# agussomacal/ROMHighContrast

Measured on AMD Instinct MI355X. Metric: snapshot_solves_per_sec, higher is better.
Workload: dtype f64

## Files before the change

### romhighcontrast_amd/csrc/rom_fem_dev.h

```cpp
#pragma once
#include "rom_fem_plan.h"
#include "rom_mma.h"

struct FemDev {
  int nrb, ncb, N, n1, n1p, nr, nc, nGp, nGa, T, nslots, kblk, npre, nrhs, nexp, ncross, xb0;
  long long dim;
  const double* pool;
  const int* alist;
  const int* aoff;
  int tile_stream;
  const int* pairs;
  int npairs;
  const double* pool_acc;
  const int* wmeta;
  int wp0[5];
  int s1_t0, s1_nterm, s1_ndr;
  const int* s1_items;
  const int* s1_citems;
  const GenTerm* terms;
  const double* Bt;
  const double* P;
  const double* vec;
  const RhsTerm* rhs;
  const PreEdge* pre;
// ... 45 lines not shown
};


FemDev make_dev(const rom_fem* f);

constexpr int S1_COEF_BYTES = 4 * COEF_MAX * 8, S1_WAVE_BYTES = (40 * 64 + 64 * 4 + 64 + 64 + 3 * 64 * 4) * 8;
constexpr int S1_ITEM_PASSES = 4;
constexpr int S1_DENSE_BYTES = 64 * 64 * 8;
constexpr int S1_LDS_BYTES = S1_COEF_BYTES + 4 * S1_WAVE_BYTES + S1_DENSE_BYTES;

__global__ void k_repack_table(const double* __restrict__ G, int ld, int nseg, int n1, int orient, double* __restrict__ Gs);
struct ExtThresholds { unsigned short thr[8]; };
__global__ void k_mask_table(double* __restrict__ G, int ld, int n1, ExtThresholds th);
__global__ void k_build_A0(double* A0, const double* Qp, const double* rho, int n1, int n1p, int N);
__global__ void k_rhs(FemDev f, const double* __restrict__ a);
__global__ void k_coef(FemDev f, const double* __restrict__ a);
__global__ void k_expand(FemDev f, const double* __restrict__ a, int Mc, double* __restrict__ U, long long row0);
__global__ void k_back_pre(FemDev f, const double* __restrict__ a, int Mc);
template <int NS>
__global__ void k_diag_update(FemDev f, const double* __restrict__ a, int slot, int Mc);
__global__ void k_diag_factor(FemDev f, int slot, int j);
__global__ void k_solve1(FemDev f, const double* __restrict__ a, int Mc);
template <int NS>
__global__ void k_factor_panel(FemDev f, const double* __restrict__ a, int j, int Mc);
__global__ void k_backsolve(FemDev f);
__global__ void k_edge_transform(FemDev f, int Mc);
__global__ void k_extend(FemDev f, const double* __restrict__ a, int Mc, double* __restrict__ U, long long row0, const int* __restrict__ blocks, int pw_log2);
struct X128Args {
  int blocks[X128_BLOCKS];
  BlockSide sides[X128_BLOCKS];
};

template <bool FLAT>
__global__ void k_extend128(FemDev f, X128Args xa, const double* __restrict__ a, int Mc, double* __restrict__ U, long long row0, int with_expand, int sys_fast);
__device__ inline void load4_any(const double* __restrict__ p, double v[4]) {
  if (p) {
    v[0] = p[0]; v[1] = p[1]; v[2] = p[2]; v[3] = p[3];
  } else {
    v[0] = v[1] = v[2] = v[3] = 0.0;
  }
}

__device__ inline void expand_tile(const FemDev& f, int Mc, double* __restrict__ U, long long row0, double* lds,
                                   int bx, int by, int bz) {
  if (bz == f.nexp) {
    if (bx != 0) return;
    for (int idx = threadIdx.x; idx < 64 * f.nscat; idx += 256) {
      const int m = by * 64 + idx / f.nscat, v = f.scat[idx % f.nscat];
      if (m < Mc) U[(row0 + m) * f.dim + f.vmap[v]] = f.y[size_t(m) * f.nGp + v];
    }
    return;
  }
  const WavePos wp;
  const ExpEdge ee = f.exp[bz];
  const int srow = stage_row(), sseg = stage_seg();
  const int mA = by * 64 + srow;
  const double* pA = mA < Mc ? f.y + size_t(mA) * f.nGp + ee.zpos + sseg : nullptr;
  const double* pB = f.P + (size_t(ee.ptab) * f.n1p + bx * 64 + srow) * f.n1p + sseg;
  const int kover = ee.zpos < f.nGa ? max(ee.zpos + ee.nch * BK - f.nGa, 0) : 0;
  Acc acc;
  acc_zero(acc);
  gemm_loop(
      ee.nch,
      [&](int ch, double* v) {
        load4_any(pA ? pA + ch * BK : nullptr, v);
        if (kover > 0 && ch == ee.nch - 1) {
#pragma unroll
// ... 33 lines not shown
```

### romhighcontrast_amd/csrc/rom_fem_kernels.hip

```cpp
#include "rom_fem_dev.h"

__global__ void k_build_A0(double* A0, const double* Qp, const double* rho, int n1, int n1p, int N) {
  size_t idx = blockIdx.x * size_t(blockDim.x) + threadIdx.x;
  size_t total = size_t(n1) * n1 * n1p;
  if (idx >= total) return;
  int m = int(idx % n1p);
  size_t ij = idx / n1p;
  int j = int(ij % n1) + 1, i = int(ij / n1) + 1;
  A0[idx] = (m < n1) ? Qp[size_t(j - 1) * n1p + m] * rho[size_t(m) * (N + 1) + i] : 0.0;
}

__global__ void k_repack_table(const double* __restrict__ G, int ld, int nseg, int n1, int orient, double* __restrict__ Gs) {
  const long long idx = blockIdx.x * (long long)blockDim.x + threadIdx.x;
  const long long hrows = (long long)n1 * n1;
  if (idx >= (long long)nseg * hrows * 8) return;
  const int kk = int(idx & 7);
  const long long rp = (idx >> 3) % hrows, seg = (idx >> 3) / hrows;
  const long long row = orient ? (rp % n1) * n1 + rp / n1 : rp;
  const int k = int(seg) * 8 + kk;
  Gs[idx] = k < ld ? G[row * ld + k] : 0.0;
}

__global__ void k_mask_table(double* __restrict__ G, int ld, int n1, ExtThresholds th) {
  const long long idx = blockIdx.x * (long long)blockDim.x + threadIdx.x;
// ... 1436 lines not shown
  const bool odd = wp.lane & 1;
  const int cfirst = acc_col(wp, odd ? 1 : 0) - (odd ? 1 : 0);
  const int ii = i0 + (cfirst >> pw_log2) - 1, jj = j0 + (cfirst & (pw - 1)) - 1;
  const bool v0 = ii < n1 && jj < n1, v1 = ii < n1 && jj + 1 < n1;
  const long long gidx = (long long)(p * N + ii) * f.nc + (q * N + jj);
  double w_own[2];
#pragma unroll
  for (int jb = 0; jb < 2; ++jb) {
    const int cidx = acc_col(wp, jb);
    const int wi = i0 + (cidx >> pw_log2) - 1, wj = j0 + (cidx & (pw - 1)) - 1;
    w_own[jb] = (wi < n1 && wj < n1) ? f.W[wi * n1 + wj] : 0.0;
  }
#pragma unroll
  for (int i = 0; i < 2; ++i)
#pragma unroll
    for (int g = 0; g < 4; ++g) {
      const int m = blockIdx.y * 64 + acc_row(wp, i, g);
      const double sc = scs[acc_row(wp, i, g)];
      const double x0 = acc.c[i][0][g] + sc * w_own[0], x1 = acc.c[i][1][g] + sc * w_own[1];
      const double got = lane_swap1(odd ? x0 : x1);
      if (m >= Mc) continue;
      double* dst = U + (row0 + m) * f.dim + gidx;
      const double lo = odd ? got : x0, hi = odd ? x1 : got;
      if (v1) *reinterpret_cast<double2_u*>(dst) = double2_u{lo, hi};
      else if (v0) dst[0] = lo;
    }
}



constexpr int X128_SLOT = 4 * 128 * 64;
static_assert(sizeof(FemDev) + sizeof(X128Args) + 64 <= 4096, "k_extend128's arguments must fit the kernel argument segment");

__device__ inline int x128_skip(const ExtSide& s, int d) {
  int n = 0;
#pragma unroll
  for (int j = 0; j < EXT_THRESHOLDS; ++j) n += d >= int(s.thr[j]) ? 1 : 0;
  return n;
}

template <bool FLAT>
__global__ __launch_bounds__(512, 2) void k_extend128(FemDev f, X128Args xa, const double* __restrict__ a, int Mc,
                                                      double* __restrict__ U, long long row0, int with_expand,
                                                      int sys_fast) {
  __shared__ __align__(16) char lds_bytes[2 * X128_SLOT];
  __shared__ double scs[128];
  double* const lds = reinterpret_cast<double*>(lds_bytes);
  const int n1 = f.n1, N = f.N;
  const int nct = (n1 + 127) / 128;
  const int nvert = n1 * n1;
  const int ntile = FLAT ? (nvert + 127) / 128 : n1 * nct;
  int bx, by, ngy;
  if (sys_fast > 0) {
    bx = int(blockIdx.x) / sys_fast; by = int(blockIdx.x) % sys_fast; ngy = sys_fast;
  } else if (sys_fast < 0) {
    ngy = -sys_fast;
    const int unit = int(blockIdx.x) / (8 * ngy), r = int(blockIdx.x) % (8 * ngy);
    bx = unit * 8 + (r & 7); by = r >> 3;
  } else {
    bx = int(blockIdx.x); by = int(blockIdx.y); ngy = int(gridDim.y);
  }
  if (bx >= ntile + with_expand) return;
  if (bx >= ntile) {
    static_assert(STAGE_TOTAL * sizeof(double) <= 2 * X128_SLOT, "expansion staging must fit");
    const int nx = f.n1p / 64, ny = (Mc + 63) / 64;
    const int item = (bx - ntile) + with_expand * (by + ngy * blockIdx.z);
    if (threadIdx.x >= 256) return;
    if (item < nx * ny * (f.nexp + 1)) expand_tile(f, Mc, U, row0, lds, item % nx, (item / nx) % ny, item / (nx * ny));
    return;
  }
  const int bz = blockIdx.z;
  {
    const unsigned lin = __builtin_amdgcn_readfirstlane(blockIdx.x + gridDim.x * (blockIdx.y + gridDim.y * bz));
    if (lin >= 256u && lin < 512u)
      for (int i = 0; i < 2; ++i) __builtin_amdgcn_s_sleep(127);
  }
  const int b = xa.blocks[bz];
  const int p = b / f.ncb, q = b % f.ncb;
  const BlockSide sd = xa.sides[bz];
  const int iv = bx / nct + 1;
  const int jv0 = 128 * (bx % nct) + 1;
  const int vt0 = 128 * bx;
  const int lane = threadIdx.x & 63, w = __builtin_amdgcn_readfirstlane(threadIdx.x >> 6), wr = w >> 2, wc = w & 3;
  constexpr int NJ = 2;
  const int fr = lane & 15, kq = lane >> 4;
  double my_sc = 0.0;
  if (threadIdx.x < 128) {
    const int m = by * 128 + threadIdx.x;
    if (m < Mc) my_sc = f.y[size_t(m) * f.nGp + f.sblk0 + b];
  }
  double w_own[NJ];
#pragma unroll
  for (int j = 0; j < NJ; ++j) {
    if (FLAT) {
      const int v = vt0 + wc * (16 * NJ) + j * 16 + fr;
      w_own[j] = v < nvert ? f.W[v] : 0.0;
    } else {
      const int jj = jv0 + wc * (16 * NJ) + j * 16 + fr;
      w_own[j] = jj <= n1 ? f.W[(iv - 1) * n1 + (jj - 1)] : 0.0;
    }
  }
  int dist0, dist1, dist2, dist3;
  if (FLAT) {
    const int vend = min(vt0 + 127, nvert - 1), i_lo = vt0 / n1, i_hi = vend / n1;
    const bool one_row = i_lo == i_hi;
    dist0 = i_lo + 1;
    dist1 = N - (i_hi + 1);
    dist2 = one_row ? vt0 - i_lo * n1 + 1 : 1;
    dist3 = one_row ? N - (vend - i_hi * n1 + 1) : 1;
  } else {
    dist0 = iv;
    dist1 = N - iv;
    dist2 = jv0;
    dist3 = N - min(jv0 + 127, n1);
  }
#define X_SEGS(S_) min(2 * sd.s[S_].nch, (sd.s[S_].r + 1 + 7) / 8)
  const int sk0 = sd.s[0].mode == 2 ? min(x128_skip(sd.s[0], dist0), X_SEGS(0) - 1) : 0;
  const int sk1 = sd.s[1].mode == 2 ? min(x128_skip(sd.s[1], dist1), X_SEGS(1) - 1) : 0;
  const int sk2 = sd.s[2].mode == 2 ? min(x128_skip(sd.s[2], dist2), X_SEGS(2) - 1) : 0;
  const int sk3 = sd.s[3].mode == 2 ? min(x128_skip(sd.s[3], dist3), X_SEGS(3) - 1) : 0;
  const int cnt0 = sd.s[0].mode == 2 ? X_SEGS(0) - sk0 : 0;
  const int cnt1 = sd.s[1].mode == 2 ? X_SEGS(1) - sk1 : 0;
  const int cnt2 = sd.s[2].mode == 2 ? X_SEGS(2) - sk2 : 0;
  const int cnt3 = sd.s[3].mode == 2 ? X_SEGS(3) - sk3 : 0;
#undef X_SEGS
  const int nseg = cnt0 + cnt1 + cnt2 + cnt3;
  const int tot = (nseg + 1) / 2;
  const unsigned fx = unsigned((kq >> 1) ^ (fr >> 2));
  const unsigned fa0 = unsigned(fr * 64) + (fx << 4) + unsigned(kq & 1) * 8u;
  const unsigned fa1 = unsigned(fr * 64) + ((fx ^ 2u) << 4) + unsigned(kq & 1) * 8u;
#define X_FRAGS(SLOT_, KKI_, AF_, BF_)                                                                             \
  do {                                                                                                             \
    const char* pf_ = lds_bytes + (SLOT_) * X128_SLOT + (((KKI_)&1) ? fa1 : fa0);                                  \
    const char* pa_ = pf_ + ((KKI_) >> 1) * 8192 + wr * 4096;                                                      \
    const char* pb_ = pf_ + 16384 + ((KKI_) >> 1) * 8192 + wc * (1024 * NJ);                                       \
    _Pragma("unroll") for (int i_ = 0; i_ < 4; ++i_) AF_[i_] = *reinterpret_cast<const double*>(pa_ + i_ * 1024);  \
    _Pragma("unroll") for (int i_ = 0; i_ < NJ; ++i_) BF_[i_] = *reinterpret_cast<const double*>(pb_ + i_ * 1024); \
  } while (0)
  const unsigned lds0 = unsigned(size_t((__attribute__((address_space(3))) char*)lds_bytes));
  const unsigned du16 = unsigned(((lane & 3) ^ ((lane >> 4) & 3)) * 16);
  const unsigned ybytes_row = unsigned(f.nGp) * 8u;
  const int m0 = by * 128;
  unsigned voA[2];
  int vi[2], vj[2];
#pragma unroll
  for (int g = 0; g < 2; ++g) {
    const int rl = 32 * (w & 3) + 16 * g + (lane >> 2);
    voA[g] = unsigned(max(0, min(rl, Mc - 1 - m0))) * ybytes_row + du16;
    if (FLAT) {
      const int v = min(vt0 + rl, nvert - 1);
      vi[g] = v / n1 + 1;
      vj[g] = v % n1 + 1;
    } else {
      vi[g] = iv;
      vj[g] = min(jv0 + rl, n1);
    }
  }
  const char* const ybase = reinterpret_cast<const char*>(f.y) + size_t(min(m0, Mc - 1)) * ybytes_row;
  const char* const gsbase = reinterpret_cast<const char*>(f.Gs);
  const size_t seg_stride = size_t(n1) * n1 * 64;
  const char* const zbase = reinterpret_cast<const char*>(f.W + size_t(n1) * n1);
  const unsigned voZ = unsigned(lane) * 16u;
  int c_side = -1, c_left = 0, c_segs = nseg;
  const char* pA = zbase;
  const char* pB = zbase;
  unsigned voB[2] = {0, 0};
#define X_NEXT_SIDE()                                                                                              \
  do {                                                                                                             \
// ... 1 lines not shown
      ++c_side;                                                                                                    \
      c_left = c_side == 0 ? cnt0 : c_side == 1 ? cnt1 : c_side == 2 ? cnt2 : cnt3;                                \
    } while (c_left == 0 && c_side < 3);                                                                           \
    const int off_ = c_side == 0 ? sd.s[0].off : c_side == 1 ? sd.s[1].off : c_side == 2 ? sd.s[2].off : sd.s[3].off; \
    const int gseg_ = c_side == 0 ? sd.s[0].gseg : c_side == 1 ? sd.s[1].gseg : c_side == 2 ? sd.s[2].gseg : sd.s[3].gseg; \
     \
         \
    const int ci_ = c_side == 1 ? -n1 : n1, cj_ = c_side == 3 ? -1 : 1;                                             \
    const int k0_ = c_side == 1 ? n1 * n1 - 1 : c_side == 3 ? -n1 + n1 : -n1 - 1;                                   \
    const int sk_ = c_side == 0 ? sk0 : c_side == 1 ? sk1 : c_side == 2 ? sk2 : sk3;         \
    pA = ybase + size_t(off_) * 8 + size_t(sk_) * 64;                                                              \
    pB = gsbase + size_t(gseg_) * 8 + size_t(sk_) * seg_stride;                                                    \
    voB[0] = unsigned(ci_ * vi[0] + cj_ * vj[0] + k0_) * 64u + du16;                                               \
    voB[1] = unsigned(ci_ * vi[1] + cj_ * vj[1] + k0_) * 64u + du16;                                               \
  } while (0)
#define X_DMA(LDS_, BASE_, VOFF_)                                                                                  \
  asm volatile("s_mov_b32 m0, %0\n\tglobal_load_lds_dwordx4 %1, %2" ::"s"(__builtin_amdgcn_readfirstlane(LDS_)),   \
               "v"(VOFF_), "s"(x128_uniform(BASE_))                                                                \
               : "memory", "m0")
#define X_ISSUE_HALF(SLOT_, H_, MINE_)                                                                             \
  do {                                                                                                             \
    const unsigned sb_ = lds0 + unsigned(SLOT_) * X128_SLOT + (H_) * 8192 + unsigned(w & 3) * 2048;                \
    if (c_segs > 0) {                                                                                              \
      if (MINE_) {                                                                                                 \
        X_DMA(sb_, pA, voA[0]);                                                                                    \
        X_DMA(sb_ + 1024, pA, voA[1]);                                                                             \
        X_DMA(sb_ + 16384, pB, voB[0]);                                                                            \
        X_DMA(sb_ + 16384 + 1024, pB, voB[1]);                                                                     \
      }                                                                                                            \
      pA += 64;                                                                                                    \
      pB += seg_stride;                                               \
      --c_segs;                                                                                                    \
      if (--c_left == 0 && c_segs > 0) X_NEXT_SIDE();                                                              \
    } else if (MINE_) {                                                 \
      X_DMA(sb_, zbase, voZ);                                                                                      \
      X_DMA(sb_ + 1024, zbase, voZ);                                                                               \
      X_DMA(sb_ + 16384, zbase, voZ);                                                                              \
      X_DMA(sb_ + 16384 + 1024, zbase, voZ);                                                                       \
    }                                                                                                              \
  } while (0)
  d4_t acc[4][NJ];
#pragma unroll
  for (int i = 0; i < 4; ++i)
#pragma unroll
    for (int j = 0; j < NJ; ++j) acc[i][j] = d4_t{0.0, 0.0, 0.0, 0.0};
  if (tot > 0) {
    X_NEXT_SIDE();
    X_ISSUE_HALF(0, 0, w < 4);
    X_ISSUE_HALF(0, 1, w < 4);
    asm volatile("s_waitcnt vmcnt(0)\n\ts_barrier" ::: "memory");
    double af[2][4], bf[2][NJ];
    X_FRAGS(0, 0, af[0], bf[0]);
    for (int ch = 0; ch < tot; ++ch) {
      const int slot = ch & 1;
      if (ch + 1 < tot) {
        const bool mine = (w >> 2) == ((ch + 1) & 1);
        X_ISSUE_HALF(slot ^ 1, 0, mine);
        X_ISSUE_HALF(slot ^ 1, 1, mine);
      }
#pragma unroll
      for (int kki = 0; kki < 4; ++kki) {
        const int pb = kki & 1;
        if (kki < 3) X_FRAGS(slot, kki + 1, af[pb ^ 1], bf[pb ^ 1]);
#pragma unroll
        for (int i = 0; i < 4; ++i)
#pragma unroll
          for (int j = 0; j < NJ; ++j) acc[i][j] = __builtin_amdgcn_mfma_f64_16x16x4f64(af[pb][i], bf[pb][j], acc[i][j], 0, 0, 0);
      }
      {
        asm volatile("s_waitcnt vmcnt(0)\n\ts_barrier" ::: "memory");
      }
      if (ch + 1 < tot) X_FRAGS(slot ^ 1, 0, af[0], bf[0]);
    }
  }
#undef X_ISSUE_HALF
#undef X_DMA
#undef X_NEXT_SIDE
#undef X_FRAGS
#ifndef ROMHC_EPI_PRIO
#define ROMHC_EPI_PRIO 3
#endif
#ifndef X128_STORE_POLICY
#define X128_STORE_POLICY ""
#endif
  __builtin_amdgcn_s_setprio(ROMHC_EPI_PRIO);
  if (threadIdx.x < 128) scs[threadIdx.x] = my_sc;
  __syncthreads();
  const bool odd = lane & 1;
  constexpr int NHP = NJ / 2;
  char* sp[NHP];
  long long d1[NHP] = {};
  unsigned long long k16[NHP], k8[NHP], k8b[NHP];
  {
    char* const rowp = reinterpret_cast<char*>(U) + size_t(row0 + m0 + wr * 64 + kq) * size_t(f.dim) * 8;
#pragma unroll
    for (int hp = 0; hp < NHP; ++hp) {
      const int t = wc * (16 * NJ) + (2 * hp + (odd ? 1 : 0)) * 16 + fr - (odd ? 1 : 0);
      long long off0, off1;
      bool ok0, ok1;
      if (FLAT) {
        const int v = vt0 + t, i0 = v / n1, j0 = v - i0 * n1;
        off0 = (long long)(p * N + i0) * f.nc + q * N + j0;
        off1 = j0 + 1 < n1 ? off0 + 1 : (long long)(p * N + i0 + 1) * f.nc + q * N;
        ok0 = v < nvert;
        ok1 = v + 1 < nvert;
      } else {
        const int jcol = jv0 + t;
        off0 = (long long)(p * N + iv - 1) * f.nc + q * N - 1 + jcol;
        off1 = off0 + 1;
        ok0 = jcol <= n1;
        ok1 = jcol + 1 <= n1;
      }
      const bool straddle = FLAT && off1 != off0 + 1;
      k16[hp] = __builtin_amdgcn_ballot_w64(ok1 && !straddle);
      k8[hp] = __builtin_amdgcn_ballot_w64(ok0 && (!ok1 || straddle));
      k8b[hp] = __builtin_amdgcn_ballot_w64(ok1 && straddle);
      sp[hp] = rowp + off0 * 8;
      d1[hp] = (off1 - off0) * 8;
    }
  }
  const long long step = 4ll * f.dim * 8;
  const bool full = m0 + 128 <= Mc;
  const int mrow = m0 + wr * 64 + kq;
#pragma unroll
  for (int i = 0; i < 4; ++i)
#pragma unroll
    for (int g = 0; g < 4; ++g) {
      const double sc = scs[wr * 64 + i * 16 + kq + 4 * g];
      unsigned long long in = ~0ull;
      if (!full) in = __builtin_amdgcn_ballot_w64(mrow + i * 16 + 4 * g < Mc);
#pragma unroll
      for (int hp = 0; hp < NHP; ++hp) {
        const double x0 = acc[i][2 * hp][g] + sc * w_own[2 * hp], x1 = acc[i][2 * hp + 1][g] + sc * w_own[2 * hp + 1];
        const double got = lane_swap1(odd ? x0 : x1);
        const double2_u pr = double2_u{odd ? got : x0, odd ? x1 : got};
        const unsigned long long m16 = x128_uniform(k16[hp] & in), m8 = x128_uniform(k8[hp] & in), m8b = x128_uniform(k8b[hp] & in);
        unsigned long long sv;
        asm volatile("s_mov_b64 %0, exec\n\ts_mov_b64 exec, %1\n\tglobal_store_dwordx4 %2, %3, off" X128_STORE_POLICY "\n\ts_mov_b64 exec, %0"
                     : "=&s"(sv)
                     : "s"(m16), "v"(sp[hp]), "v"(pr));
        if (m8 != 0)
          asm volatile("s_mov_b64 %0, exec\n\ts_mov_b64 exec, %1\n\tglobal_store_dwordx2 %2, %3, off" X128_STORE_POLICY "\n\ts_mov_b64 exec, %0"
                       : "=&s"(sv)
                       : "s"(m8), "v"(sp[hp]), "v"(pr.x));
        if (FLAT && m8b != 0)
          asm volatile("s_mov_b64 %0, exec\n\ts_mov_b64 exec, %1\n\tglobal_store_dwordx2 %2, %3, off" X128_STORE_POLICY "\n\ts_mov_b64 exec, %0"
                       : "=&s"(sv)
                       : "s"(m8b), "v"(sp[hp] + d1[hp]), "v"(pr.y));
        sp[hp] += step;
      }
    }
}
template __global__ void k_extend128<false>(FemDev, X128Args, const double*, int, double*, long long, int, int);
template __global__ void k_extend128<true>(FemDev, X128Args, const double*, int, double*, long long, int, int);

__global__ void k_scatter_interface(FemDev f, int Mc, double* __restrict__ U, long long row0) {
  int i = blockIdx.x * blockDim.x + threadIdx.x;
  int m = blockIdx.y;
  if (i >= f.nscat || m >= Mc) return;
  const int v = f.scat[i];
  U[(row0 + m) * f.dim + f.vmap[v]] = f.y[size_t(m) * f.nGp + v];
}

__global__ void k_assemble_stencil(FemDev f, const double* __restrict__ a, int M, double* __restrict__ diag,
                                   double* __restrict__ east, double* __restrict__ north) {
  __shared__ double am[64];
  const int m = blockIdx.y;
  for (int i = threadIdx.x; i < f.kblk; i += blockDim.x) am[i] = a[size_t(m) * f.kblk + i];
  __syncthreads();
  long long idx = blockIdx.x * (long long)blockDim.x + threadIdx.x;
  if (idx >= f.dim) return;
  int r = int(idx / f.nc) + 1, c = int(idx % f.nc) + 1;
  int N = f.N, ncb = f.ncb;
  double k00 = am[((r - 1) / N) * ncb + (c - 1) / N];
  double k01 = am[((r - 1) / N) * ncb + c / N];
  double k10 = am[(r / N) * ncb + (c - 1) / N];
  double k11 = am[(r / N) * ncb + c / N];
  diag[size_t(m) * f.dim + idx] = ((k00 + k01) + k10) + k11;
  if (c < f.nc) east[size_t(m) * f.nr * (f.nc - 1) + size_t(r - 1) * (f.nc - 1) + (c - 1)] = -(k11 + k01) / 2;
  if (r < f.nr) north[size_t(m) * (f.nr - 1) * f.nc + size_t(r - 1) * f.nc + (c - 1)] = -(k11 + k10) / 2;
}
```

### romhighcontrast_amd/csrc/rom_fem_plan.h

```cpp
#pragma once
#include <string>
#include <vector>

#include "romhc_internal.h"

constexpr int COEF_MAX = 64;
#ifndef PAIR_RING_
#define PAIR_RING_ 8
#endif
constexpr int PAIR_RING = PAIR_RING_;
constexpr int DENSE_GROUPS_MAX = 8;
constexpr int EXT_ZERO_PAGE = 256;
constexpr int EXT_THRESHOLDS = 7;
constexpr long double EXT_TRUNC_CUT = 1e-18L;
constexpr int X128_BLOCKS = 16;

__host__ __device__ inline int h0_row(int s, int i, int j, int N, int n1) {
  int ii, jj;
  switch (s) {
    case 0: ii = i; jj = j; break;
    case 1: ii = N - i; jj = j; break;
    case 2: ii = j; jj = i; break;
    default: ii = N - j; jj = i; break;
  }
  return (ii - 1) * n1 + (jj - 1);
}

struct FemSwitches {
  bool no_preelim, no_compress, no_lowrank_ext, no_ext_lr, verbose;
  long double compress_tol;
  bool no_ext_trunc;
};

struct FemPlan {
  int nrb, ncb, N, n1, n1p, nr, nc, nG, nGp, nGa, nred, ncross, xb0, T, nslots, n_all_edges, npre_all;
  int64_t dim;
  int spos0, nsc, npairs = 0, wp0[5] = {}, ncoef, ncf, nctask, ndg, ndi, n_edges, lr_nch;
  bool fused1 = false;
  std::vector<double> pool, pool_acc, dmat, Ptab, Bt, Qp, rho, Wz, g_red, vecs, cm;
  std::vector<GenTerm> terms;
  std::vector<TileDesc> desc;
  std::vector<int> alist, aoff, pairs, wmeta, s1_items, s1_citems, dweight, ditem_group, ditem_k, kmax, item_group, item_k, item_cf;
  std::vector<int> ctask, xred, scb, kptr, kpair, colptr, colrow, colti, vmap, scat, lr_blocks, gen_blocks, epos;
  std::vector<DenseGroup> dgroups;
  std::vector<RhsTerm> rhs_terms;
  std::vector<PreEdge> pre_edges;
  std::vector<ExpEdge> exps;
  std::vector<CoefGroup> groups;
  std::vector<BlockSide> sides;
  struct GemmG {
    std::vector<double> Bh; long long off; int rp;
    int r = 0;
    std::vector<int> entry, seg0;
    std::vector<long double> W;
    unsigned short thr[8] = {0xffff, 0xffff, 0xffff, 0xffff, 0xffff, 0xffff, 0xffff, 0xffff};
    double cut = 0;
  };
  struct Repack { long long goff, gsoff; int ld, nseg, orient; };
// ... 9 lines not shown
```

### romhighcontrast_amd/csrc/rom_fem_setup.hip

```cpp
#include <algorithm>
#include <cstdlib>
#include <cstring>
#include <memory>

#include "rom_fem_dev.h"

#ifdef ROMHC_AB
static const char* ab_env(const char* name) { return getenv(name); }
#else
static const char* ab_env(const char*) { return nullptr; }
#endif

FemDev make_dev(const rom_fem* f) {
  FemDev d;
  d.nrb = f->nrb; d.ncb = f->ncb; d.N = f->N; d.n1 = f->n1; d.n1p = f->n1p; d.nr = f->nr; d.nc = f->nc;
  d.nGp = f->nGp; d.nGa = f->nGa; d.T = f->T; d.nslots = f->nslots; d.kblk = f->nrb * f->ncb; d.npre = f->npre;
  d.nrhs = f->nrhs; d.nexp = f->nexp; d.ncross = f->ncross; d.xb0 = f->xb0; d.dim = f->dim;
  d.pool = f->d_pool; d.alist = f->d_alist; d.aoff = f->d_aoff; d.tile_stream = f->sw_no_tile_stream ? 0 : 1;
  d.pairs = f->d_pairs; d.npairs = f->npairs; d.pool_acc = f->d_pool_acc; d.wmeta = f->d_wmeta;
  for (int i = 0; i < 5; ++i) d.wp0[i] = f->wp0[i];
  d.s1_t0 = d.s1_nterm = d.s1_ndr = 0;
  if (f->fused1 && !f->desc.empty()) {
    d.s1_t0 = f->desc[0].t0; d.s1_nterm = f->desc[0].t1 - f->desc[0].t0; d.s1_ndr = f->desc[0].ndr;
  }
// ... 120 lines not shown
  f->ctx = ctx;
  f->nrb = nrb; f->ncb = ncb; f->N = N; f->n1 = p.n1; f->n1p = p.n1p; f->nr = p.nr; f->nc = p.nc; f->dim = p.dim;
  f->nG = p.nG; f->nGp = p.nGp; f->nGa = p.nGa; f->nred = p.nred; f->ncross = p.ncross; f->xb0 = p.xb0; f->T = p.T;
  f->nslots = p.nslots; f->npre = int(p.pre_edges.size()); f->nexp = int(p.exps.size()); f->nrhs = int(p.rhs_terms.size());
  f->spos0 = p.spos0; f->nsc = p.nsc; f->n_all_edges = p.n_all_edges; f->npairs = p.npairs; f->fused1 = p.fused1;
  for (int i = 0; i < 5; ++i) f->wp0[i] = p.wp0[i];
  f->ncoef = p.ncoef; f->ncf = p.ncf; f->nctask = p.nctask; f->ndg = p.ndg; f->ndi = p.ndi; f->n_edges = p.n_edges;
  f->n_lr_blocks = int(p.lr_blocks.size()); f->n_gen_blocks = int(p.gen_blocks.size()); f->lr_nch = p.lr_nch;
  f->nscat = int(p.scat.size()); f->ext_flops = p.ext_flops; f->flops_solve = p.flops_solve; f->bytes_solve = p.bytes_solve;
  f->desc = p.desc; f->slot_of = p.slot_of; f->kptr = p.kptr; f->kpair = p.kpair; f->colptr = p.colptr; f->colrow = p.colrow;
  f->colti = p.colti; f->diag_slot = p.diag_slot; f->sides = p.sides; f->ranks = p.ranks; f->lr_blocks_host = p.lr_blocks;
#define ROM_UPLOAD(member, vec) ROM_TRY(upload(ctx->stream, f->tables, &f->member, p.vec))
  ROM_UPLOAD(d_pool, pool);         ROM_UPLOAD(d_terms, terms);           ROM_UPLOAD(d_desc, desc);
  ROM_UPLOAD(d_alist, alist);       ROM_UPLOAD(d_aoff, aoff);             ROM_UPLOAD(d_pairs, pairs);
  ROM_UPLOAD(d_pool_acc, pool_acc); ROM_UPLOAD(d_wmeta, wmeta);           ROM_UPLOAD(d_s1_items, s1_items);
  ROM_UPLOAD(d_s1_citems, s1_citems); ROM_UPLOAD(d_dgroups, dgroups);     ROM_UPLOAD(d_dweight, dweight);
  ROM_UPLOAD(d_ditem_group, ditem_group); ROM_UPLOAD(d_ditem_k, ditem_k); ROM_UPLOAD(d_dmat, dmat);
  ROM_UPLOAD(d_P, Ptab);            ROM_UPLOAD(d_Bt, Bt);                 ROM_UPLOAD(d_Qp, Qp);
  ROM_UPLOAD(d_kmax, kmax);         ROM_UPLOAD(d_W, Wz);                  ROM_UPLOAD(d_g, g_red);
  ROM_UPLOAD(d_vec, vecs);          ROM_UPLOAD(d_rhs, rhs_terms);         ROM_UPLOAD(d_pre, pre_edges);
  ROM_UPLOAD(d_exp, exps);          ROM_UPLOAD(d_groups, groups);         ROM_UPLOAD(d_cm, cm);
  ROM_UPLOAD(d_item_group, item_group); ROM_UPLOAD(d_item_k, item_k);     ROM_UPLOAD(d_item_cf, item_cf);
  ROM_UPLOAD(d_ctask, ctask);       ROM_UPLOAD(d_xred, xred);             ROM_UPLOAD(d_scb, scb);
  ROM_UPLOAD(d_kptr, kptr);         ROM_UPLOAD(d_kpair, kpair);           ROM_UPLOAD(d_colptr, colptr);
  ROM_UPLOAD(d_colrow, colrow);     ROM_UPLOAD(d_colti, colti);           ROM_UPLOAD(d_sides, sides);
  ROM_UPLOAD(d_vmap, vmap);         ROM_UPLOAD(d_scat, scat);             ROM_UPLOAD(d_lr_blocks, lr_blocks);
  ROM_UPLOAD(d_gen_blocks, gen_blocks); ROM_UPLOAD(d_epos, epos);
#undef ROM_UPLOAD
  ROM_TRY(build_extension_tables(f, p));
  if (f->fused1)
    ROM_HIP(hipFuncSetAttribute(reinterpret_cast<const void*>(k_solve1), hipFuncAttributeMaxDynamicSharedMemorySize, S1_LDS_BYTES));
  f->sw_no_fused = getenv("ROMHC_NO_FUSED") != nullptr;
  f->sw_no_ext128 = getenv("ROMHC_NO_EXT128") != nullptr;
#ifdef ROMHC_AB
  f->sw_x128_sys_fast = ab_env("ROMHC_X128_SYS_FAST") ? atoi(ab_env("ROMHC_X128_SYS_FAST")) : -1;
  f->sw_no_fold = ab_env("ROMHC_NO_FOLD_EXPAND") != nullptr;
  f->sw_coef_global = ab_env("ROMHC_COEF_GLOBAL") != nullptr;
  f->sw_no_tile_pairs = ab_env("ROMHC_NO_TILE_PAIRS") != nullptr;
  f->sw_no_tile_stream = ab_env("ROMHC_NO_TILE_STREAM") != nullptr;
  f->sw_ext_flat = ab_env("ROMHC_EXT_FLAT") ? (atoi(ab_env("ROMHC_EXT_FLAT")) != 0 ? 1 : 0) : -1;
#endif
  *out = guard.release();
  return ROM_OK;
}
```

### romhighcontrast_amd/csrc/rom_fem_solve.hip

```cpp
#include <algorithm>
#include <cstdlib>
#include <cstring>

#include "rom_fem_dev.h"

extern "C" int rom_fem_dims(rom_fem* f, int* nr, int* nc, int64_t* dim, int* n_interface, int* n_tiles) {
  ROM_CHECK(f, "null fem");
  if (nr) *nr = f->nr;
  if (nc) *nc = f->nc;
  if (dim) *dim = f->dim;
  if (n_interface) *n_interface = f->nG;
  if (n_tiles) *n_tiles = f->nslots;
  return ROM_OK;
}

extern "C" int rom_fem_load_vector_host(rom_fem* f, double* B) {
  ROM_CHECK(f && B, "bad arguments");
  double area = (1.0 / f->N) * (1.0 / f->N);
  double v = 0.0;
  v += area / 6;
  v += area / 3;
  v += area / 3;
  v += area / 6;
  for (int64_t i = 0; i < f->dim; ++i) B[i] = v;
// ... 138 lines not shown
      k_back_pre<<<dim3(f->n1p / 64, (Mc + 63) / 64, f->npre), 256, 0, st>>>(d, am, Mc);
    }
  }
  {
    const int nij = f->n1 * f->n1;
    if (nij > 0) {
      if (f->n_edges > 0) {
        ROM_PROF(ctx, "edge_transform", Mc * 2.0 * f->n_edges * double(f->n1p) * f->n1p, 16.0 * Mc * f->n_edges * f->n1p);
        k_edge_transform<<<dim3(f->n1p / 64, (Mc + 63) / 64, f->n_edges), 256, 0, st>>>(d, Mc);
      }
      const int npatch = ((f->n1 + 3) / 4) * ((f->n1 + 15) / 16);
      const double fl_ext = (f->ext_flops - 2.0 * f->n_edges * double(f->n1p) * f->n1p) * Mc / kblk;
      if (f->n_gen_blocks > 0) {
        dim3 grid(npatch, (Mc + 63) / 64, f->n_gen_blocks);
        ROM_PROF(ctx, "extend", fl_ext * f->n_gen_blocks, 8.0 * Mc * double(f->n_gen_blocks) * nij);
        k_extend<<<grid, 256, 0, st>>>(d, am, Mc, U, row, d.gen_blocks, 4);
      }
      if (f->n_lr_blocks > 0) {
        ROM_PROF(ctx, "extend_lr", fl_ext * f->n_lr_blocks, 8.0 * Mc * double(f->n_lr_blocks) * nij);
        if (wide) {
          const int mt = (Mc + 127) / 128;
          const int items = (f->n1p / 64) * ((Mc + 63) / 64) * (f->nexp + 1);
          for (int z0 = 0; z0 < f->n_lr_blocks; z0 += X128_BLOCKS) {
            const int nz = std::min(X128_BLOCKS, f->n_lr_blocks - z0);
            X128Args xa;
            memset(&xa, 0, sizeof(xa));
            for (int z = 0; z < nz; ++z) {
              xa.blocks[z] = f->lr_blocks_host[z0 + z];
              xa.sides[z] = f->sides[xa.blocks[z]];
            }
            const int extra = fold_expand && z0 == 0 ? (items + mt * nz - 1) / (mt * nz) : 0;
            const int order = f->sw_x128_sys_fast >= 0 ? f->sw_x128_sys_fast : (f->gs_bytes >= (size_t(64) << 20) && mt >= 16 ? 1 : 0);
            const int sys_fast = order == 1 ? mt : order == 2 ? -mt : 0;
            const int nx = sys_fast < 0 ? (t128 + extra + 7) / 8 * 8 : t128 + extra;
            dim3 grid(sys_fast ? nx * mt : nx, sys_fast ? 1 : mt, nz);
            if (flat) k_extend128<true><<<grid, 512, 0, st>>>(d, xa, am, Mc, U, row, extra, sys_fast);
            else k_extend128<false><<<grid, 512, 0, st>>>(d, xa, am, Mc, U, row, extra, sys_fast);
          }
        } else {
          dim3 grid(f->n1 * ((f->n1 + 63) / 64), (Mc + 63) / 64, f->n_lr_blocks);
          k_extend<<<grid, 256, 0, st>>>(d, am, Mc, U, row, d.lr_blocks, 6);
        }
      }
    }
    if (f->nscat > 0 && !(f->nexp > 0 && f->npre == 0)) {
      ROM_PROF(ctx, "scatter_interface", 0, 16.0 * Mc * f->nscat);
      k_scatter_interface<<<dim3((f->nscat + 255) / 256, Mc), 256, 0, st>>>(d, Mc, U, row);
    }
  }
  ROM_HIP(hipGetLastError());
  return ROM_OK;
}

static int solve_batch_impl(rom_fem* f, rom_buf* a, int M, rom_buf* U, int64_t row0, bool check, rom_buf* Y = nullptr,
                            int64_t y_row0 = 0, int stages = 3) {
  ROM_CHECK(f && a && (U || !(stages & 2)), "rom_solve_batch: null argument");
  ROM_CHECK(M >= 0 && row0 >= 0 && y_row0 >= 0, "rom_solve_batch: negative M or row offset");
  const int kblk = f->nrb * f->ncb;
  ROM_CHECK(a->n >= size_t(M) * kblk, "rom_solve_batch: `a` holds %zu doubles, need %zu", a->n, size_t(M) * kblk);
  if (stages & 2)
    ROM_CHECK(U->n >= size_t(row0 + M) * f->dim, "rom_solve_batch: U holds %zu doubles, need %zu", U->n,
              size_t(row0 + M) * f->dim);
  if (Y)
    ROM_CHECK(Y->n >= size_t(y_row0 + M) * f->nGp, "rom_solve_batch: the interface-vector buffer holds %zu doubles, need %zu",
              Y->n, size_t(y_row0 + M) * f->nGp);
  if (M == 0) return ROM_OK;
  rom_ctx* ctx = f->ctx;
  ROM_HIP(hipSetDevice(ctx->device));
  size_t per_sys = (size_t(f->nslots) * 4096 + size_t(f->T) * 4096 + 2 * size_t(f->nGp)) * sizeof(double);
  int Mc_max = int(std::max<size_t>(1, std::min<size_t>(size_t(M), ctx->ws_limit / std::max<size_t>(per_sys, 1))));
// ... 152 lines not shown
```

### romhighcontrast_amd/csrc/romhc_internal.h

```cpp
#pragma once
#include <hip/hip_runtime.h>

#include <cstdarg>
#include <cstdint>
#include <cstdio>
#include <map>
#include <string>
#include <vector>

#include "romhc.h"

void rom_set_error(const char* fmt, ...);

#define ROM_HIP(call)                                                                      \
  do {                                                                                     \
    hipError_t _e = (call);                                                                \
    if (_e != hipSuccess) {                                                                \
      rom_set_error("%s failed: %s (%s:%d)", #call, hipGetErrorString(_e), __FILE__, __LINE__); \
      return ROM_ERR_HIP;                                                                  \
    }                                                                                      \
  } while (0)

#define ROM_CHECK(cond, ...)      \
  do {                            \
// ... 192 lines not shown
  int* d_alist = nullptr;
  int* d_aoff = nullptr;
  int npairs = 0;
  double* d_pool_acc = nullptr;
  int* d_wmeta = nullptr;
  int wp0[5] = {};
  int* d_s1_items = nullptr;
  int* d_s1_citems = nullptr;
  int* d_kptr = nullptr;
  int* d_kpair = nullptr;
  int* d_colptr = nullptr;
  int* d_colrow = nullptr;
  int* d_colti = nullptr;
  double* d_Bt = nullptr;
  double* d_P = nullptr;
  double* d_vec = nullptr;
  RhsTerm* d_rhs = nullptr;
  PreEdge* d_pre = nullptr;
  ExpEdge* d_exp = nullptr;
  int* d_xred = nullptr;
  int* d_scb = nullptr;
  int spos0 = 0, nsc = 0, n_all_edges = 0;
  CoefGroup* d_groups = nullptr;
  double* d_cm = nullptr;
  int* d_item_group = nullptr;
  int* d_item_k = nullptr;
  int ncoef = 0;
  int* d_item_cf = nullptr;
  int* d_ctask = nullptr;
  int nctask = 0, ncf = 0;
  bool lds_optin_coef = false;
  bool fused1 = false;
  bool sw_no_fused = false, sw_no_ext128 = false, sw_no_fold = false;
  int sw_x128_sys_fast = -1;
  size_t gs_bytes = 0;
  int sw_ext_flat = -1;
  bool sw_coef_global = false;
  bool sw_no_tile_pairs = false;
  bool sw_no_tile_stream = false;
  DenseGroup* d_dgroups = nullptr;
  int* d_dweight = nullptr;
  int* d_ditem_group = nullptr;
  int* d_ditem_k = nullptr;
  double* d_dmat = nullptr;
  int ndg = 0, ndi = 0;
  int nrhs = 0;
  BlockSide* d_sides = nullptr;
  int* d_lr_blocks = nullptr;
  std::vector<int> lr_blocks_host;
  int* d_gen_blocks = nullptr;
  int n_lr_blocks = 0, n_gen_blocks = 0, lr_nch = 0;
  int* d_vmap = nullptr;
  int* d_scat = nullptr;
  int nscat = 0;
  std::vector<TileDesc> desc;
  std::vector<int> slot_of, kptr, kpair, colptr, colrow, colti, diag_slot;
  std::vector<BlockSide> sides;
  std::vector<int> ranks;
  double flops_solve = 0, bytes_solve = 0;
  void* fmap = nullptr;
  double* d_riesz = nullptr;
  double* d_green = nullptr;
  double* d_L = nullptr;
  double* d_invL = nullptr;
  double* d_y = nullptr;
  int ws_M = 0;
// ... 12 lines not shown
```

Before: 4.253 million.

## Skip dead K-halves per wave in extend128 via per-wave threshold masks

Computes skip thresholds per wave column (32 vertices) in addition to per tile, builds a bitmask of live half-segments, and lets each wave skip the LDS fragment loads and MFMAs for segments that are masked out for its own vertices. Zero-fill DMA for skipped segments is suppressed when per-wave mode is active, and the wave column order is mirrored for the second wave row, presumably to balance skipped work across SIMDs. Per-wave skipping applies only when the segment count is under 64 and can be disabled by an environment switch. It adds branchy control flow and a non-unrolled inner loop, which may hurt scheduling when little work is skipped.

```diff
diff --git a/romhighcontrast_amd/csrc/rom_fem_dev.h b/romhighcontrast_amd/csrc/rom_fem_dev.h
--- a/romhighcontrast_amd/csrc/rom_fem_dev.h
+++ b/romhighcontrast_amd/csrc/rom_fem_dev.h
@@ -101,7 +101,8 @@
 };
 
 template <bool FLAT>
-__global__ void k_extend128(FemDev f, X128Args xa, const double* __restrict__ a, int Mc, double* __restrict__ U, long long row0, int with_expand, int sys_fast);
+__global__ void k_extend128(FemDev f, X128Args xa, const double* __restrict__ a, int Mc, double* __restrict__ U, long long row0, int with_expand, int sys_fast,
+                            int wave_skip);
 __device__ inline void load4_any(const double* __restrict__ p, double v[4]) {
   if (p) {
     v[0] = p[0]; v[1] = p[1]; v[2] = p[2]; v[3] = p[3];
diff --git a/romhighcontrast_amd/csrc/rom_fem_kernels.hip b/romhighcontrast_amd/csrc/rom_fem_kernels.hip
--- a/romhighcontrast_amd/csrc/rom_fem_kernels.hip
+++ b/romhighcontrast_amd/csrc/rom_fem_kernels.hip
@@ -1492,17 +1492,10 @@
 constexpr int X128_SLOT = 4 * 128 * 64;
 static_assert(sizeof(FemDev) + sizeof(X128Args) + 64 <= 4096, "k_extend128's arguments must fit the kernel argument segment");
 
-__device__ inline int x128_skip(const ExtSide& s, int d) {
-  int n = 0;
-#pragma unroll
-  for (int j = 0; j < EXT_THRESHOLDS; ++j) n += d >= int(s.thr[j]) ? 1 : 0;
-  return n;
-}
-
 template <bool FLAT>
 __global__ __launch_bounds__(512, 2) void k_extend128(FemDev f, X128Args xa, const double* __restrict__ a, int Mc,
                                                       double* __restrict__ U, long long row0, int with_expand,
-                                                      int sys_fast) {
+                                                      int sys_fast, int wave_skip) {
   __shared__ __align__(16) char lds_bytes[2 * X128_SLOT];
   __shared__ double scs[128];
   double* const lds = reinterpret_cast<double*>(lds_bytes);
@@ -1542,6 +1535,10 @@
   const int jv0 = 128 * (bx % nct) + 1;
   const int vt0 = 128 * bx;
   const int lane = threadIdx.x & 63, w = __builtin_amdgcn_readfirstlane(threadIdx.x >> 6), wr = w >> 2, wc = w & 3;
+#ifndef X128_MIRROR
+#define X128_MIRROR 1
+#endif
+  const int wcv = X128_MIRROR && wr ? 3 - wc : wc;
   constexpr int NJ = 2;
   const int fr = lane & 15, kq = lane >> 4;
   double my_sc = 0.0;
@@ -1553,39 +1550,37 @@
 #pragma unroll
   for (int j = 0; j < NJ; ++j) {
     if (FLAT) {
-      const int v = vt0 + wc * (16 * NJ) + j * 16 + fr;
+      const int v = vt0 + wcv * (16 * NJ) + j * 16 + fr;
       w_own[j] = v < nvert ? f.W[v] : 0.0;
     } else {
-      const int jj = jv0 + wc * (16 * NJ) + j * 16 + fr;
+      const int jj = jv0 + wcv * (16 * NJ) + j * 16 + fr;
       w_own[j] = jj <= n1 ? f.W[(iv - 1) * n1 + (jj - 1)] : 0.0;
     }
   }
-  int dist0, dist1, dist2, dist3;
-  if (FLAT) {
-    const int vend = min(vt0 + 127, nvert - 1), i_lo = vt0 / n1, i_hi = vend / n1;
-    const bool one_row = i_lo == i_hi;
-    dist0 = i_lo + 1;
-    dist1 = N - (i_hi + 1);
-    dist2 = one_row ? vt0 - i_lo * n1 + 1 : 1;
-    dist3 = one_row ? N - (vend - i_hi * n1 + 1) : 1;
-  } else {
-    dist0 = iv;
-    dist1 = N - iv;
-    dist2 = jv0;
-    dist3 = N - min(jv0 + 127, n1);
-  }
-#define X_SEGS(S_) min(2 * sd.s[S_].nch, (sd.s[S_].r + 1 + 7) / 8)
-  const int sk0 = sd.s[0].mode == 2 ? min(x128_skip(sd.s[0], dist0), X_SEGS(0) - 1) : 0;
-  const int sk1 = sd.s[1].mode == 2 ? min(x128_skip(sd.s[1], dist1), X_SEGS(1) - 1) : 0;
-  const int sk2 = sd.s[2].mode == 2 ? min(x128_skip(sd.s[2], dist2), X_SEGS(2) - 1) : 0;
-  const int sk3 = sd.s[3].mode == 2 ? min(x128_skip(sd.s[3], dist3), X_SEGS(3) - 1) : 0;
-  const int cnt0 = sd.s[0].mode == 2 ? X_SEGS(0) - sk0 : 0;
-  const int cnt1 = sd.s[1].mode == 2 ? X_SEGS(1) - sk1 : 0;
-  const int cnt2 = sd.s[2].mode == 2 ? X_SEGS(2) - sk2 : 0;
-  const int cnt3 = sd.s[3].mode == 2 ? X_SEGS(3) - sk3 : 0;
-#undef X_SEGS
+  int tsk[4], wsk[4];
+  const bool has_vertices = x128_skip_counts<FLAT>(n1, N, bx, wcv, sd.s[0], sd.s[1], sd.s[2], sd.s[3], tsk, wsk);
+  const int sk0 = tsk[0], sk1 = tsk[1], sk2 = tsk[2], sk3 = tsk[3];
+  const int cnt0 = x128_segs(sd.s[0]) - sk0, cnt1 = x128_segs(sd.s[1]) - sk1;
+  const int cnt2 = x128_segs(sd.s[2]) - sk2, cnt3 = x128_segs(sd.s[3]) - sk3;
   const int nseg = cnt0 + cnt1 + cnt2 + cnt3;
   const int tot = (nseg + 1) / 2;
+  const bool per_wave = wave_skip != 0 && nseg < 64;
+  long long live = -1;
+  if (per_wave) {
+    unsigned long long m = 0;
+    int h0 = 0;
+#define X_LIVE(S_, CNT_)                                                                                           \
+  do {                       \
+    m |= ((1ull << (CNT_)) - (1ull << (wsk[S_] - tsk[S_]))) << h0;                                                  \
+    h0 += (CNT_);                                                                                                  \
+  } while (0)
+    X_LIVE(0, cnt0);
+    X_LIVE(1, cnt1);
+    X_LIVE(2, cnt2);
+    X_LIVE(3, cnt3);
+#undef X_LIVE
+    live = (long long)x128_uniform(has_vertices ? m : 0ull);
+  }
   const unsigned fx = unsigned((kq >> 1) ^ (fr >> 2));
   const unsigned fa0 = unsigned(fr * 64) + (fx << 4) + unsigned(kq & 1) * 8u;
   const unsigned fa1 = unsigned(fr * 64) + ((fx ^ 2u) << 4) + unsigned(kq & 1) * 8u;
@@ -1593,7 +1588,7 @@
   do {                                                                                                             \
     const char* pf_ = lds_bytes + (SLOT_) * X128_SLOT + (((KKI_)&1) ? fa1 : fa0);                                  \
     const char* pa_ = pf_ + ((KKI_) >> 1) * 8192 + wr * 4096;                                                      \
-    const char* pb_ = pf_ + 16384 + ((KKI_) >> 1) * 8192 + wc * (1024 * NJ);                                       \
+    const char* pb_ = pf_ + 16384 + ((KKI_) >> 1) * 8192 + wcv * (1024 * NJ);                                     \
     _Pragma("unroll") for (int i_ = 0; i_ < 4; ++i_) AF_[i_] = *reinterpret_cast<const double*>(pa_ + i_ * 1024);  \
     _Pragma("unroll") for (int i_ = 0; i_ < NJ; ++i_) BF_[i_] = *reinterpret_cast<const double*>(pb_ + i_ * 1024); \
   } while (0)
@@ -1661,7 +1656,7 @@
       pB += seg_stride;                                               \
       --c_segs;                                                                                                    \
       if (--c_left == 0 && c_segs > 0) X_NEXT_SIDE();                                                              \
-    } else if (MINE_) {                                                 \
+    } else if ((MINE_) && !per_wave) {     \
       X_DMA(sb_, zbase, voZ);                                                                                      \
       X_DMA(sb_ + 1024, zbase, voZ);                                                                               \
       X_DMA(sb_ + 16384, zbase, voZ);                                                                              \
@@ -1679,7 +1674,18 @@
     X_ISSUE_HALF(0, 1, w < 4);
     asm volatile("s_waitcnt vmcnt(0)\n\ts_barrier" ::: "memory");
     double af[2][4], bf[2][NJ];
-    X_FRAGS(0, 0, af[0], bf[0]);
+#define X_MFMAS(PB_)                                                                                               \
+  do {                                                                                                             \
+    _Pragma("unroll") for (int i = 0; i < 4; ++i)                                                                  \
+      _Pragma("unroll") for (int j = 0; j < NJ; ++j)                                                               \
+        acc[i][j] = __builtin_amdgcn_mfma_f64_16x16x4f64(af[PB_][i], bf[PB_][j], acc[i][j], 0, 0, 0);              \
+  } while (0)
+#define X_FIRST_FRAGS(SLOT_)                                                                                       \
+  do {                                                                                                             \
+    if (live & 1) X_FRAGS(SLOT_, 0, af[0], bf[0]);                                                                 \
+    else if (live & 2) X_FRAGS(SLOT_, 2, af[0], bf[0]);                                                            \
+  } while (0)
+    X_FIRST_FRAGS(0);
     for (int ch = 0; ch < tot; ++ch) {
       const int slot = ch & 1;
       if (ch + 1 < tot) {
@@ -1687,21 +1693,23 @@
         X_ISSUE_HALF(slot ^ 1, 0, mine);
         X_ISSUE_HALF(slot ^ 1, 1, mine);
       }
-#pragma unroll
-      for (int kki = 0; kki < 4; ++kki) {
-        const int pb = kki & 1;
-        if (kki < 3) X_FRAGS(slot, kki + 1, af[pb ^ 1], bf[pb ^ 1]);
-#pragma unroll
-        for (int i = 0; i < 4; ++i)
-#pragma unroll
-          for (int j = 0; j < NJ; ++j) acc[i][j] = __builtin_amdgcn_mfma_f64_16x16x4f64(af[pb][i], bf[pb][j], acc[i][j], 0, 0, 0);
-      }
+      const int h_lo = (live & 1) ? 0 : 1, h_hi = (live & 2) ? 2 : 1;
+#pragma unroll 1
+      for (int h = h_lo; h < h_hi; ++h) {
+        X_FRAGS(slot, 2 * h + 1, af[1], bf[1]);
+        X_MFMAS(0);
+        if (h + 1 < h_hi) X_FRAGS(slot, 2, af[0], bf[0]);
+        X_MFMAS(1);
+      }
+      live >>= 2;
       {
         asm volatile("s_waitcnt vmcnt(0)\n\ts_barrier" ::: "memory");
       }
-      if (ch + 1 < tot) X_FRAGS(slot ^ 1, 0, af[0], bf[0]);
-    }
-  }
+      if (ch + 1 < tot) X_FIRST_FRAGS(slot ^ 1);
+    }
+  }
+#undef X_FIRST_FRAGS
+#undef X_MFMAS
 #undef X_ISSUE_HALF
 #undef X_DMA
 #undef X_NEXT_SIDE
@@ -1724,7 +1732,7 @@
     char* const rowp = reinterpret_cast<char*>(U) + size_t(row0 + m0 + wr * 64 + kq) * size_t(f.dim) * 8;
 #pragma unroll
     for (int hp = 0; hp < NHP; ++hp) {
-      const int t = wc * (16 * NJ) + (2 * hp + (odd ? 1 : 0)) * 16 + fr - (odd ? 1 : 0);
+      const int t = wcv * (16 * NJ) + (2 * hp + (odd ? 1 : 0)) * 16 + fr - (odd ? 1 : 0);
       long long off0, off1;
       bool ok0, ok1;
       if (FLAT) {
@@ -1780,8 +1788,8 @@
       }
     }
 }
-template __global__ void k_extend128<false>(FemDev, X128Args, const double*, int, double*, long long, int, int);
-template __global__ void k_extend128<true>(FemDev, X128Args, const double*, int, double*, long long, int, int);
+template __global__ void k_extend128<false>(FemDev, X128Args, const double*, int, double*, long long, int, int, int);
+template __global__ void k_extend128<true>(FemDev, X128Args, const double*, int, double*, long long, int, int, int);
 
 __global__ void k_scatter_interface(FemDev f, int Mc, double* __restrict__ U, long long row0) {
   int i = blockIdx.x * blockDim.x + threadIdx.x;
diff --git a/romhighcontrast_amd/csrc/rom_fem_plan.h b/romhighcontrast_amd/csrc/rom_fem_plan.h
--- a/romhighcontrast_amd/csrc/rom_fem_plan.h
+++ b/romhighcontrast_amd/csrc/rom_fem_plan.h
@@ -24,6 +24,69 @@
     default: ii = N - j; jj = i; break;
   }
   return (ii - 1) * n1 + (jj - 1);
+}
+
+__host__ __device__ inline int x128_skip(const ExtSide& s, int d) {
+  int n = 0;
+#ifdef __HIP_DEVICE_COMPILE__
+#pragma unroll
+#endif
+  for (int j = 0; j < EXT_THRESHOLDS; ++j) n += d >= int(s.thr[j]) ? 1 : 0;
+  return n;
+}
+__host__ __device__ inline int x128_segs(const ExtSide& s) {
+  const int padded = 2 * s.nch, filled = (s.r + 1 + 7) / 8;
+  return s.mode == 2 ? (padded < filled ? padded : filled) : 0;
+}
+__host__ __device__ inline int x128_skip_clamped(const ExtSide& s, int d) {
+  const int n = x128_skip(s, d), last = x128_segs(s) - 1;
+  return s.mode == 2 ? (n < last ? n : last) : 0;
+}
+
+template <bool FLAT>
+__host__ __device__ inline bool x128_skip_counts(int n1, int N, int tile, int wc, const ExtSide& s0, const ExtSide& s1,
+                                                 const ExtSide& s2, const ExtSide& s3, int tsk[4], int wsk[4]) {
+  int dist0, dist1, dist2, dist3;
+  int wd0, wd1, wd2, wd3;
+  bool has;
+  if (FLAT) {
+    const int nvert = n1 * n1, vt0 = 128 * tile;
+    const int vend = vt0 + 127 < nvert - 1 ? vt0 + 127 : nvert - 1, i_lo = vt0 / n1, i_hi = vend / n1;
+    const bool one_row = i_lo == i_hi;
+    dist0 = i_lo + 1;
+    dist1 = N - (i_hi + 1);
+    dist2 = one_row ? vt0 - i_lo * n1 + 1 : 1;
+    dist3 = one_row ? N - (vend - i_hi * n1 + 1) : 1;
+    const int v0 = vt0 + 32 * wc, v1 = v0 + 31 < vend ? v0 + 31 : vend;
+    has = v0 <= vend;
+    const int w_lo = has ? v0 / n1 : i_lo, w_hi = has ? v1 / n1 : i_hi;
+    const bool w_one = w_lo == w_hi;
+    wd0 = w_lo + 1;
+    wd1 = N - (w_hi + 1);
+    wd2 = w_one ? v0 - w_lo * n1 + 1 : 1;
+    wd3 = w_one ? N - (v1 - w_hi * n1 + 1) : 1;
+  } else {
+    const int nct = (n1 + 127) / 128, iv = tile / nct + 1, jv0 = 128 * (tile % nct) + 1;
+    dist0 = iv;
+    dist1 = N - iv;
+    dist2 = jv0;
+    dist3 = N - (jv0 + 127 < n1 ? jv0 + 127 : n1);
+    const int jw = jv0 + 32 * wc;
+    has = jw <= n1;
+    wd0 = iv;
+    wd1 = N - iv;
+    wd2 = jw;
+    wd3 = N - (jw + 31 < n1 ? jw + 31 : n1);
+  }
+  tsk[0] = x128_skip_clamped(s0, dist0);
+  tsk[1] = x128_skip_clamped(s1, dist1);
+  tsk[2] = x128_skip_clamped(s2, dist2);
+  tsk[3] = x128_skip_clamped(s3, dist3);
+  wsk[0] = has ? x128_skip_clamped(s0, wd0) : tsk[0];
+  wsk[1] = has ? x128_skip_clamped(s1, wd1) : tsk[1];
+  wsk[2] = has ? x128_skip_clamped(s2, wd2) : tsk[2];
+  wsk[3] = has ? x128_skip_clamped(s3, wd3) : tsk[3];
+  return has;
 }
 
 struct FemSwitches {
diff --git a/romhighcontrast_amd/csrc/rom_fem_setup.hip b/romhighcontrast_amd/csrc/rom_fem_setup.hip
--- a/romhighcontrast_amd/csrc/rom_fem_setup.hip
+++ b/romhighcontrast_amd/csrc/rom_fem_setup.hip
@@ -176,6 +176,7 @@
     ROM_HIP(hipFuncSetAttribute(reinterpret_cast<const void*>(k_solve1), hipFuncAttributeMaxDynamicSharedMemorySize, S1_LDS_BYTES));
   f->sw_no_fused = getenv("ROMHC_NO_FUSED") != nullptr;
   f->sw_no_ext128 = getenv("ROMHC_NO_EXT128") != nullptr;
+  f->sw_no_ext_wave_skip = getenv("ROMHC_NO_EXT_WAVE_SKIP") != nullptr;
 #ifdef ROMHC_AB
   f->sw_x128_sys_fast = ab_env("ROMHC_X128_SYS_FAST") ? atoi(ab_env("ROMHC_X128_SYS_FAST")) : -1;
   f->sw_no_fold = ab_env("ROMHC_NO_FOLD_EXPAND") != nullptr;
diff --git a/romhighcontrast_amd/csrc/rom_fem_solve.hip b/romhighcontrast_amd/csrc/rom_fem_solve.hip
--- a/romhighcontrast_amd/csrc/rom_fem_solve.hip
+++ b/romhighcontrast_amd/csrc/rom_fem_solve.hip
@@ -194,10 +194,11 @@
             const int extra = fold_expand && z0 == 0 ? (items + mt * nz - 1) / (mt * nz) : 0;
             const int order = f->sw_x128_sys_fast >= 0 ? f->sw_x128_sys_fast : (f->gs_bytes >= (size_t(64) << 20) && mt >= 16 ? 1 : 0);
             const int sys_fast = order == 1 ? mt : order == 2 ? -mt : 0;
+            const int wave_skip = f->sw_no_ext_wave_skip ? 0 : 1;
             const int nx = sys_fast < 0 ? (t128 + extra + 7) / 8 * 8 : t128 + extra;
             dim3 grid(sys_fast ? nx * mt : nx, sys_fast ? 1 : mt, nz);
-            if (flat) k_extend128<true><<<grid, 512, 0, st>>>(d, xa, am, Mc, U, row, extra, sys_fast);
-            else k_extend128<false><<<grid, 512, 0, st>>>(d, xa, am, Mc, U, row, extra, sys_fast);
+            if (flat) k_extend128<true><<<grid, 512, 0, st>>>(d, xa, am, Mc, U, row, extra, sys_fast, wave_skip);
+            else k_extend128<false><<<grid, 512, 0, st>>>(d, xa, am, Mc, U, row, extra, sys_fast, wave_skip);
           }
         } else {
           dim3 grid(f->n1 * ((f->n1 + 63) / 64), (Mc + 63) / 64, f->n_lr_blocks);
diff --git a/romhighcontrast_amd/csrc/romhc_internal.h b/romhighcontrast_amd/csrc/romhc_internal.h
--- a/romhighcontrast_amd/csrc/romhc_internal.h
+++ b/romhighcontrast_amd/csrc/romhc_internal.h
@@ -248,6 +248,7 @@
   bool lds_optin_coef = false;
   bool fused1 = false;
   bool sw_no_fused = false, sw_no_ext128 = false, sw_no_fold = false;
+  bool sw_no_ext_wave_skip = false;
   int sw_x128_sys_fast = -1;
   size_t gs_bytes = 0;
   int sw_ext_flat = -1;
```

Result: faster. 4.456 million, median of 6 (+4.8%).
